# kwea123/nerf_pl

Hardware: NVIDIA H100
Metric: ray-samples/sec (coarse+fine) (higher is better)
Workload: dtype f16 (fp32 accumulate, fp32 encoding/compositing)

## Files before the change

include/nerf_pl_b200.h:

```cpp
#ifndef NERF_PL_B200_H_
#define NERF_PL_B200_H_

#include <stddef.h>
#include <stdint.h>

#ifdef __cplusplus
extern "C" {
#endif

#define NERFB200_ABI_VERSION 3

#define NERFB200_EINVAL (-1)
#define NERFB200_EUNSUPPORTED (-2)
#define NERFB200_EDEVICE (-3)

int nerfb200_abi_version(void);
const char* nerfb200_last_error(void);

size_t nerfb200_packed_bytes(void);
int nerfb200_pack_weights(const float* const params[24], void* packed, void* stream);
int nerfb200_pack_weights_pair(const float* const params_a[24], void* packed_a, const float* const params_b[24],
                               void* packed_b, void* stream);

typedef struct nerfb200_render_args {
// ... 68 lines not shown
int nerfb200_nerf_forward_train(const float* x, int64_t n, int64_t x_stride, const void* packed, void* ws, float* out,
                                void* stream);
int nerfb200_nerf_backward(const float* g_out, int64_t n, const void* packed, const float* const params[24], void* ws,
                           float* const grads[24], void* stream);

int nerfb200_query_sigma(const float* xyz, int64_t n, int64_t xyz_stride, const void* packed, float* sigma,
                         void* stream);

int nerfb200_mse_psnr(const float* rgb_coarse, const float* rgb_fine, const float* target, int64_t n_rays,
                      float* out4, void* stream);

int nerfb200_embed(const float* x, int64_t n, int32_t n_freqs, float* out, void* stream);

int nerfb200_searchsorted(const float* a, const float* v, int64_t* out, int64_t nrow_a,
                          int64_t nrow_v, int32_t ncol_a, int32_t ncol_v, int32_t side_right,
                          void* stream);

int nerfb200_sample_pdf(const float* bins, const float* weights, const float* u, int64_t n_rays,
                        int32_t n_weights, int32_t n_u, float* out, void* stream);

int nerfb200_composite(const float* sigmas, const float* rgbs, const float* z_vals,
                       const float* dirs, const float* noise, float noise_std, int32_t white_back,
                       int64_t n_rays, int32_t n_samples, float* weights, float* rgb, float* depth,
                       float* opacity, void* stream);

int nerfb200_generate_rays(int32_t H, int32_t W, float focal, const float c2w_host[12], float near, float far,
                           int32_t ndc, float* rays, void* stream);

int nerfb200_to_uint8(const float* src, int64_t n, uint8_t* dst, void* stream);

int64_t nerfb200_launch_count(void);
int nerfb200_check_status(void);
int nerfb200_sm_count(void);

#ifdef __cplusplus
}
#endif
#endif
```

nerf_pl_b200/_lib.py:

```python
from __future__ import annotations

import ctypes
import os
import subprocess
import threading
from ctypes import POINTER, c_char_p, c_float, c_int32, c_int64, c_size_t, c_void_p

_HERE = os.path.dirname(os.path.abspath(__file__))
CSRC = os.path.join(_HERE, "csrc")
LIB_PATH = os.path.join(_HERE, "libnerf_pl_b200.so")
if os.environ.get("NERFB200_LIB"):
    LIB_PATH = os.path.abspath(os.environ["NERFB200_LIB"])
SOURCES = ["capi.cu"]
HEADERS = ["ptx.cuh", "layout.h", "mlp_engine.cuh", "render_kernel.cuh", "aux_kernels.cuh", "bwd_kernels.cuh"]
NVCC_FLAGS = [
    "-gencode", "arch=compute_90a,code=sm_90a",
    "-O3", "-lineinfo", "-std=c++17",
    "--shared", "-Xcompiler", "-fPIC",
    "-diag-suppress", "550",
]

EXPORTS = [
    "nerfb200_abi_version",
    "nerfb200_last_error",
    "nerfb200_packed_bytes",
    "nerfb200_pack_weights",
    "nerfb200_pack_weights_pair",
    "nerfb200_render_rays",
    "nerfb200_render_rays_host",
    "nerfb200_nerf_forward",
    "nerfb200_nerf_train_workspace_bytes",
    "nerfb200_nerf_train_workspace_init",
    "nerfb200_nerf_forward_train",
    "nerfb200_nerf_backward",
    "nerfb200_embed",
    "nerfb200_searchsorted",
    "nerfb200_sample_pdf",
    "nerfb200_composite",
    "nerfb200_query_sigma",
    "nerfb200_mse_psnr",
    "nerfb200_train_workspace_bytes",
    "nerfb200_train_workspace_init",
    "nerfb200_render_backward",
    "nerfb200_adam_step",
    "nerfb200_generate_rays",
    "nerfb200_to_uint8",
    "nerfb200_launch_count",
    "nerfb200_check_status",
    "nerfb200_sm_count",
]

class RenderArgs(ctypes.Structure):

    _fields_ = [
        ("rays", c_void_p),
        ("n_rays", c_int64),
        ("ray_stride", c_int64),
        ("packed_coarse", c_void_p),
        ("packed_fine", c_void_p),
        ("n_samples", c_int32),
        ("n_importance", c_int32),
        ("use_disp", c_int32),
        ("perturb", c_float),
        ("noise_std", c_float),
        ("white_back", c_int32),
        ("test_time", c_int32),
        ("perturb_rand", c_void_p),
        ("noise_coarse", c_void_p),
        ("u_rand", c_void_p),
        ("noise_fine", c_void_p),
        ("rgb_coarse", c_void_p),
        ("depth_coarse", c_void_p),
        ("opacity_coarse", c_void_p),
        ("rgb_fine", c_void_p),
        ("depth_fine", c_void_p),
        ("opacity_fine", c_void_p),
        ("z_fine", c_void_p),
        ("weights_coarse", c_void_p),
        ("weights_fine", c_void_p),
        ("status", c_void_p),
        ("max_ctas", c_int32),
        ("z_coarse", c_void_p),
# ... 76 lines not shown
    lib.nerfb200_composite.argtypes = [c_void_p, c_void_p, c_void_p, c_void_p, c_void_p, c_float,
                                       c_int32, c_int64, c_int32, c_void_p, c_void_p, c_void_p,
                                       c_void_p, c_void_p]
    lib.nerfb200_query_sigma.argtypes = [c_void_p, c_int64, c_int64, c_void_p, c_void_p, c_void_p]
    lib.nerfb200_query_sigma.restype = c_int32
    lib.nerfb200_nerf_train_workspace_bytes.argtypes = [c_int64]
    lib.nerfb200_nerf_train_workspace_bytes.restype = c_size_t
    lib.nerfb200_nerf_train_workspace_init.argtypes = [c_void_p, c_size_t, c_int64, c_void_p]
    lib.nerfb200_nerf_train_workspace_init.restype = c_int32
    lib.nerfb200_nerf_forward_train.argtypes = [c_void_p, c_int64, c_int64, c_void_p, c_void_p, c_void_p, c_void_p]
    lib.nerfb200_nerf_forward_train.restype = c_int32
    lib.nerfb200_nerf_backward.argtypes = [c_void_p, c_int64, c_void_p, POINTER(c_void_p), c_void_p, POINTER(c_void_p),
                                           c_void_p]
    lib.nerfb200_nerf_backward.restype = c_int32
    lib.nerfb200_train_workspace_bytes.argtypes = [c_int64, c_int32, c_int32]
    lib.nerfb200_train_workspace_bytes.restype = c_size_t
    lib.nerfb200_train_workspace_init.argtypes = [c_void_p, c_size_t, c_int64, c_int32, c_int32, c_void_p]
    lib.nerfb200_train_workspace_init.restype = c_int32
    lib.nerfb200_render_backward.argtypes = [POINTER(BackwardArgs), c_void_p]
    lib.nerfb200_render_backward.restype = c_int32
    lib.nerfb200_adam_step.argtypes = [c_int32, POINTER(c_void_p), POINTER(c_void_p), POINTER(c_void_p), POINTER(c_void_p),
                                       POINTER(c_int64), c_float, c_float, c_float, c_float, c_float, c_int64, c_void_p]
    lib.nerfb200_adam_step.restype = c_int32
    lib.nerfb200_mse_psnr.argtypes = [c_void_p, c_void_p, c_void_p, c_int64, c_void_p, c_void_p]
    lib.nerfb200_mse_psnr.restype = c_int32
    lib.nerfb200_generate_rays.argtypes = [c_int32, c_int32, c_float, POINTER(c_float), c_float, c_float, c_int32,
                                           c_void_p, c_void_p]
    lib.nerfb200_generate_rays.restype = c_int32
    lib.nerfb200_to_uint8.argtypes = [c_void_p, c_int64, c_void_p, c_void_p]
    lib.nerfb200_to_uint8.restype = c_int32
    lib.nerfb200_check_status.restype = c_int32
    lib.nerfb200_launch_count.restype = c_int64
    lib.nerfb200_sm_count.restype = c_int32
    for name in ("nerfb200_pack_weights", "nerfb200_pack_weights_pair", "nerfb200_render_rays", "nerfb200_render_rays_host",
                 "nerfb200_nerf_forward", "nerfb200_embed", "nerfb200_searchsorted",
                 "nerfb200_sample_pdf", "nerfb200_composite"):
        getattr(lib, name).restype = c_int32


def load() -> ctypes.CDLL:
    global _lib
    with _lock:
        if _lib is None:
            if not os.path.exists(LIB_PATH):
                raise RuntimeError(
                    f"{LIB_PATH} is missing: run `python -c 'import __graft_entry__ as g; g.build()'` "
                    "(nerf_pl_b200 has no CPU fallback)")
            lib = ctypes.CDLL(LIB_PATH)
            _declare(lib)
            if lib.nerfb200_abi_version() != 3:
                raise RuntimeError("libnerf_pl_b200.so ABI version mismatch")
            _lib = lib
    return _lib


class NerfB200Error(RuntimeError):
    pass


def check(rc: int, what: str) -> None:
    if rc == 0:
        return
    msg = load().nerfb200_last_error().decode("utf-8", "replace")
    if rc in (-1, -2):
        raise ValueError(f"{what}: {msg}")
    raise NerfB200Error(f"{what}: {msg} (code {rc})")
# ... 1 lines not shown
```

nerf_pl_b200/csrc/capi.cu:

```cuda
#include <atomic>
#include <cstdio>
#include <cstdlib>
#include <cmath>
#include <cstring>
#include <mutex>
#include <vector>

#include "../../include/nerf_pl_b200.h"
#include "aux_kernels.cuh"
#include "bwd_kernels.cuh"

using namespace nerfb200;

namespace {

thread_local char g_err[512] = "";
std::atomic<long long> g_launches{0};

int fail(int code, const char* fmt, const char* detail = "") {
  std::snprintf(g_err, sizeof(g_err), fmt, detail);
  return code;
}
int cuda_fail(cudaError_t e, const char* where) {
  std::snprintf(g_err, sizeof(g_err), "%s: %s (%s)", where, cudaGetErrorString(e), cudaGetErrorName(e));
  return static_cast<int>(e);
}
#define CUDA_TRY(expr, where)                          \
  do {                                                 \
    cudaError_t e_ = (expr);                           \
    if (e_ != cudaSuccess) return cuda_fail(e_, where); \
  } while (0)

struct DeviceInfo {
  int sm_count = 0;
  int cc_major = 0, cc_minor = 0;
  bool attrs_set = false;
  int* status = nullptr;
  volatile int* status_host = nullptr;
  long long* timeline = nullptr;
};

struct EnvSwitches {
  unsigned flags = 0;
  int max_ctas = 0;
  int wg_plan = 1;
  int wg_copy = 32768;
  unsigned wg_exp = 0;
  int no_zero_copy = 0;
  EnvSwitches() {
    if (const char* v = std::getenv("NERFB200_NO_ZERO_COPY")) no_zero_copy = std::atoi(v);
    if (const char* v = std::getenv("NERFB200_WG_EXP")) wg_exp = static_cast<unsigned>(std::atoi(v));
    if (const char* v = std::getenv("NERFB200_WG_PLAN")) wg_plan = std::atoi(v);
    if (const char* v = std::getenv("NERFB200_WG_COPY")) wg_copy = std::atoi(v);
    if (const char* f = std::getenv("NERFB200_FLAGS")) flags = static_cast<unsigned>(std::strtoul(f, nullptr, 0));
    if (const char* mc = std::getenv("NERFB200_MAX_CTAS")) max_ctas = std::atoi(mc);
  }
};
const EnvSwitches& env_switches() {
  static const EnvSwitches e;
  return e;
}
std::mutex g_mu;
DeviceInfo g_dev[64];

int device_info(DeviceInfo** out) {
  int dev = 0;
  CUDA_TRY(cudaGetDevice(&dev), "cudaGetDevice");
  if (dev < 0 || dev >= 64) return fail(NERFB200_EDEVICE, "device ordinal out of range%s");
  std::lock_guard<std::mutex> lk(g_mu);
  DeviceInfo& d = g_dev[dev];
  if (d.sm_count == 0) {
    CUDA_TRY(cudaDeviceGetAttribute(&d.sm_count, cudaDevAttrMultiProcessorCount, dev), "attr sm");
    CUDA_TRY(cudaDeviceGetAttribute(&d.cc_major, cudaDevAttrComputeCapabilityMajor, dev), "attr cc");
    CUDA_TRY(cudaDeviceGetAttribute(&d.cc_minor, cudaDevAttrComputeCapabilityMinor, dev), "attr cc minor");
  }
  if (d.cc_major != 9 || d.cc_minor != 0) return fail(NERFB200_EDEVICE, "nerf_pl_b200 needs an sm_90 (H100) device%s");
  if (!d.attrs_set) {
    CUDA_TRY(cudaFuncSetAttribute(render_rays_kernel<false>, cudaFuncAttributeMaxDynamicSharedMemorySize,
                                  static_cast<int>(kSmemTotal)), "smem attr render");
    CUDA_TRY(cudaFuncSetAttribute(render_rays_kernel<true>, cudaFuncAttributeMaxDynamicSharedMemorySize,
                                  static_cast<int>(kSmemTotal)), "smem attr render(save)");
    CUDA_TRY(cudaFuncSetAttribute(mlp_forward_kernel<false>, cudaFuncAttributeMaxDynamicSharedMemorySize,
                                  static_cast<int>(kSmemTotal)), "smem attr mlp");
    CUDA_TRY(cudaFuncSetAttribute(mlp_forward_kernel<true>, cudaFuncAttributeMaxDynamicSharedMemorySize,
                                  static_cast<int>(kSmemTotal)), "smem attr mlp(save)");
    CUDA_TRY(cudaFuncSetAttribute(chain_bwd_kernel<false>, cudaFuncAttributeMaxDynamicSharedMemorySize,
                                  static_cast<int>(kChSmemTotal)), "smem attr chain");
    CUDA_TRY(cudaFuncSetAttribute(chain_bwd_kernel<true>, cudaFuncAttributeMaxDynamicSharedMemorySize,
                                  static_cast<int>(kChSmemTotal)), "smem attr chain (probe)");
    CUDA_TRY(cudaFuncSetAttribute(wgrad_kernel, cudaFuncAttributeMaxDynamicSharedMemorySize,
                                  static_cast<int>(kWgSmemTotal)), "smem attr wgrad");
    CUDA_TRY(cudaFuncSetAttribute(sample_pdf_kernel, cudaFuncAttributeMaxDynamicSharedMemorySize,
                                  static_cast<int>(kPdfWarps * (kPdfMaxWeights + 1) * sizeof(float))), "smem attr sample_pdf");
    int* hs = nullptr;
    CUDA_TRY(cudaHostAlloc(&hs, sizeof(int), cudaHostAllocMapped), "status alloc");
    *hs = 0;
    CUDA_TRY(cudaHostGetDevicePointer(&d.status, hs, 0), "status device pointer");
    d.status_host = hs;
    d.attrs_set = true;
  }
  *out = &d;
  return 0;
}

int check_sticky_status(DeviceInfo* d) {
  if (d->status_host == nullptr) return 0;
  const int st = *d->status_host;
  if (st == 0) return 0;
  *d->status_host = 0;
  if (st == 102)
    std::snprintf(g_err, sizeof(g_err), "an earlier training backward reported device status 102: a per-sample "
                  "gradient exceeded the fp16 range of its layer's scale, its weight gradients are wrong");
  else
    std::snprintf(g_err, sizeof(g_err), "an earlier nerf_pl_b200 kernel reported device status %d", st);
  return NERFB200_EDEVICE;
}

int check_render_shapes(const nerfb200_render_args* a) {
  if (a == nullptr) return fail(NERFB200_EINVAL, "args is NULL%s");
  if (a->n_rays < 0) return fail(NERFB200_EINVAL, "n_rays < 0%s");
  if (a->n_samples != 32 && a->n_samples != 64 && a->n_samples != 128)
    return fail(NERFB200_EUNSUPPORTED, "N_samples must be 32, 64 or 128%s");
  if (a->n_importance < 0 || (a->n_importance % 32) != 0)
    return fail(NERFB200_EUNSUPPORTED, "N_importance must be a multiple of 32%s");
  if (a->n_samples + a->n_importance > kMaxSf)
    return fail(NERFB200_EUNSUPPORTED, "N_samples + N_importance must be <= 192%s");
// ... 347 lines not shown
  add(slot(kJ1), kWgSlotFloats, ns(kJ1), g[0], linv + 8, 256, 63, 256, 63, 0, 1);
  add(slot(kJ1) + 65536, kWgSlotFloats, ns(kJ1), g[1], linv + 8, 1, 256, 256, 256, 0);
  const int hidden[6] = {kJ2, kJ3, kJ4, kJ6, kJ7, kJ8};
  const int layer[6] = {2, 3, 4, 6, 7, 8};
  for (int i = 0; i < 6; ++i) {
    const float* inv = linv + (9 - layer[i]);
    add(slot(hidden[i]), kWgSlotFloats, ns(hidden[i]), g[2 * (layer[i] - 1)], inv, 256, 256, 256, 256, 0, 1);
    add(slot(hidden[i]) + 65536, kWgSlotFloats, ns(hidden[i]), g[2 * (layer[i] - 1) + 1], inv, 1, 256, 256, 256, 0);
  }
  add(slot(kJ5a), kWgSlotFloats, ns(kJ5a), g[8], linv + 4, 256, 63, 256, 319, 0, 1);
  add(slot(kJ5b), kWgSlotFloats, ns(kJ5b), g[8], linv + 4, 256, 256, 256, 319, 63, 1);
  add(slot(kJ5a) + 65536, kWgSlotFloats, ns(kJ5a), g[9], linv + 4, 1, 256, 256, 256, 0);
  add(slot(kJ9), kWgSlotFloats, ns(kJ9), L.gWp[ps], linv, 128, 256, 128, 256, 0, 1);
  add(slot(kJ9) + 65536, kWgSlotFloats, ns(kJ9), L.gbp[ps], linv, 1, 128, 128, 128, 0);
  add(L.head_part[ps] + kHeadPartSigW, kHeadPartFloats, L.head_grid, g[20], nullptr, 1, 256, 256, 256, 0);
  add(L.head_part[ps] + kHeadPartSigB, kHeadPartFloats, L.head_grid, g[21], nullptr, 1, 1, 1, 1, 0);
  add(L.head_part[ps] + kHeadPartRgbW, kHeadPartFloats, L.head_grid, g[22], nullptr, 1, 384, 384, 384, 0);
  add(L.head_part[ps] + kHeadPartRgbB, kHeadPartFloats, L.head_grid, g[23], nullptr, 1, 3, 3, 3, 0);
  if (L.n_kinds == kNumJobKindsMlp)
    add(slot(kJDir), kWgSlotFloats, ns(kJDir), g[18], linv, 128, 27, 128, 283, 256, 1);
  else
    add(L.dir_part[ps], 128 * 27, kDirSlices, g[18], nullptr, 128, 27, 27, 283, 256);
}

}

extern "C" {

int nerfb200_abi_version(void) { return NERFB200_ABI_VERSION; }
const char* nerfb200_last_error(void) { return g_err; }
size_t nerfb200_packed_bytes(void) { return kPackedBytes; }
int64_t nerfb200_launch_count(void) { return g_launches.load(); }

int nerfb200_sm_count(void) {
  int dev = 0, n = 0;
  if (cudaGetDevice(&dev) != cudaSuccess) return 0;
  if (cudaDeviceGetAttribute(&n, cudaDevAttrMultiProcessorCount, dev) != cudaSuccess) return 0;
  return n;
}

static int fill_pack_params(PackParams* pp, const float* const params[24], void* packed) {
  if (!params || !packed) return fail(NERFB200_EINVAL, "pack_weights: NULL argument%s");
  if (reinterpret_cast<uintptr_t>(packed) & 15) return fail(NERFB200_EINVAL, "packed must be 16-byte aligned%s");
  for (int i = 0; i < kNumParams; ++i) {
    if (!params[i]) return fail(NERFB200_EINVAL, "pack_weights: NULL parameter tensor%s");
    pp->p[i] = params[i];
  }
  pp->out = static_cast<uint8_t*>(packed);
  pp->bwd_bf16 = kBwdBf16 ? 1 : 0;
  return 0;
}

static int launch_pack(const PackParams2& pp2, int n_nets, void* stream) {
  const long long total = kHalfRegionBytes / 2 + kF32Count + static_cast<long long>(kNumSlicesBwd) * 256 * 64;
  const int threads = 256;
  const int blocks = static_cast<int>((total + threads - 1) / threads);
  pack_weights_kernel<<<dim3(blocks, n_nets), threads, 0, static_cast<cudaStream_t>(stream)>>>(pp2);
  g_launches++;
  CUDA_TRY(cudaGetLastError(), "pack_weights launch");
  return 0;
}

int nerfb200_pack_weights(const float* const params[24], void* packed, void* stream) {
  PackParams2 pp2;
  int rc = fill_pack_params(&pp2.net[0], params, packed);
  if (rc) return rc;
// ... 62 lines not shown
    make_train_layout(&L, static_cast<uint8_t*>(a->train_workspace), a->n_rays, a->n_samples, a->n_importance, d->sm_count);
    p.train = 1;
    p.tr[0] = L.pass[0];
    p.tr[1] = L.pass[1];
    if (!p.z_coarse) p.z_coarse = L.pass[0].z;
    else return fail(NERFB200_EINVAL, "z_coarse is owned by the workspace in training mode%s");
    if (a->n_importance > 0) {
      if (p.z_fine) return fail(NERFB200_EINVAL, "z_fine is owned by the workspace in training mode%s");
      p.z_fine = L.pass[1].z;
    }
    if (a->target) {
      p.target = a->target;
      p.loss_out = a->loss_out;
      p.loss_part = L.loss_part;
      p.loss_counter = L.loss_counter;
    }
  }
  p.flags = env_switches().flags;
  p.timeline = nullptr;
#ifdef NERFB200_TIMELINE
  if (p.flags & 2u) {
    if (!d->timeline) {
      CUDA_TRY(cudaMalloc(&d->timeline, 3 * kTlMax * 2 * sizeof(long long)), "timeline alloc");
    }
    CUDA_TRY(cudaMemsetAsync(d->timeline, 0, 3 * kTlMax * 2 * sizeof(long long), static_cast<cudaStream_t>(stream)), "timeline memset");
    p.timeline = d->timeline;
  }
#endif
  const int n_groups = (p.n_rays + 1) / 2;
  int ctas = d->sm_count;
  if (a->max_ctas > 0 && a->max_ctas < ctas) ctas = a->max_ctas;
  if (env_switches().max_ctas > 0 && env_switches().max_ctas < ctas) ctas = env_switches().max_ctas;
  if (n_groups < ctas) ctas = n_groups;
  if (save)
    render_rays_kernel<true><<<ctas, kRenderThreads, kSmemTotal, static_cast<cudaStream_t>(stream)>>>(p);
  else
    render_rays_kernel<false><<<ctas, kRenderThreads, kSmemTotal, static_cast<cudaStream_t>(stream)>>>(p);
  g_launches++;
  CUDA_TRY(cudaGetLastError(), "render_rays launch");
  return 0;
}

int nerfb200_render_rays_host(const nerfb200_render_args* h, void* stream_v) {
  int rc = check_render_shapes(h);
  if (rc) return rc;
  if (h->n_rays == 0) return 0;
  cudaStream_t stream = static_cast<cudaStream_t>(stream_v);
  if (h->train_workspace || h->target || h->z_coarse)
    return fail(NERFB200_EINVAL, "render_rays_host: train_workspace / target / z_coarse are device-only%s");
  {
    bool all_mapped = true;
    auto mapped = [&](const void* p, const void** dp) -> bool {
      *dp = nullptr;
      if (!p) return true;
      cudaPointerAttributes attr;
      if (cudaPointerGetAttributes(&attr, p) != cudaSuccess) { (void)cudaGetLastError(); return false; }
      if ((attr.type == cudaMemoryTypeHost || attr.type == cudaMemoryTypeDevice || attr.type == cudaMemoryTypeManaged) &&
          attr.devicePointer != nullptr) {
        *dp = attr.devicePointer;
        return true;
      }
      return false;
    };
    nerfb200_render_args a = *h;
    const void* dp = nullptr;
#define NERFB200_MAP(field, type)                                          \
    all_mapped = all_mapped && mapped(h->field, &dp);                      \
    a.field = static_cast<type>(const_cast<void*>(dp));
    NERFB200_MAP(rays, const float*)
    NERFB200_MAP(perturb_rand, const float*)
    NERFB200_MAP(noise_coarse, const float*)
// ... 597 lines not shown
```

nerf_pl_b200/csrc/mlp_engine.cuh:

```cuda
#pragma once
#include <cuda_fp16.h>

#include "layout.h"
#include "ptx.cuh"

namespace nerfb200 {

constexpr int kConsumerWGs = 2;
constexpr int kConsumerThreads = kConsumerWGs * 128;
constexpr int kConsumerWarp0 = 4;
constexpr int kProducerWarp = 0;
constexpr int kThreads = (1 + kConsumerWGs) * 128;
constexpr int kRegsAux = 56;
constexpr int kRegsConsumer = 224;
static_assert(kRegsAux + 2 * kRegsConsumer <= 3 * 168, "setmaxnreg budget");
constexpr int kWgBar0 = 4;
#ifndef NERFB200_STAGES
#define NERFB200_STAGES 3
#endif
constexpr int kStages = NERFB200_STAGES;

constexpr uint32_t kSmemEnc = 0;
constexpr uint32_t kSmemRing = 16384;
constexpr uint32_t kSmemEnc1 = kSmemRing + kStages * kSliceBytes256;
constexpr uint32_t kSmemConsts = kSmemEnc1 + 16384;
constexpr uint32_t kConstFloats = kF32WDirPart;
constexpr uint32_t kConstRegion = 24576;
constexpr uint32_t kSmemScratch = kSmemConsts + kConstRegion;
static_assert(2 * kConstFloats * 4 <= kConstRegion, "constants of two networks must fit");
static_assert(kSmemEnc1 % 1024 == 0 && kSmemConsts % 1024 == 0, "SWIZZLE_128B tiles need 1024-byte alignment");
constexpr uint32_t kSmemTotal = 232448;
constexpr uint32_t kScratchBytes = kSmemTotal - kSmemScratch;

struct Barriers {
  uint64_t full[kStages];
  uint64_t empty[kStages];
};
static_assert(sizeof(Barriers) % 16 == 0, "Barriers must keep 16-byte alignment of what follows");

struct RingState {
  uint32_t stage = 0, phase = 0;
  __device__ __forceinline__ void advance() {
    if (++stage == kStages) { stage = 0; phase ^= 1; }
  }
};

__device__ __forceinline__ bool engine_setup(uint8_t* smem, Barriers* bars) {
  if ((smem_u32(smem) & 1023u) != 0) return false;
  if (threadIdx.x == 0) {
    for (int i = 0; i < kStages; ++i) {
      mbar_init(smem_u32(&bars->full[i]), 1);
      mbar_init(smem_u32(&bars->empty[i]), kConsumerWGs * 4);
    }
    fence_mbar_init();
  }
  __syncthreads();
  return true;
}

__device__ __forceinline__ void load_consts(uint8_t* smem, int slot, const uint8_t* __restrict__ blob) {
  if (blob == nullptr) return;
  const float4* src = reinterpret_cast<const float4*>(blob + kHalfRegionBytes);
  float4* dst = reinterpret_cast<float4*>(smem + kSmemConsts) + slot * (kConstFloats / 4);
  for (uint32_t i = threadIdx.x; i < kConstFloats / 4; i += blockDim.x) dst[i] = __ldg(src + i);
}
__device__ __forceinline__ const float* consts_ptr(uint8_t* smem, int slot) {
  return reinterpret_cast<const float*>(smem + kSmemConsts) + slot * kConstFloats;
}

__device__ __forceinline__ void produce_tile(RingState& rs, uint8_t* smem, Barriers* bars,
                                             const uint8_t* __restrict__ blob, bool sigma_only,
                                             bool dir_slice) {
  const int n256 = sigma_only ? kNumSlicesSigmaOnly : kNumSlices256;
  for (int i = 0; i < n256; ++i) {
    mbar_wait(smem_u32(&bars->empty[rs.stage]), rs.phase ^ 1, 1);
    const uint32_t full = smem_u32(&bars->full[rs.stage]);
    const uint32_t dst = smem_u32(smem + kSmemRing + rs.stage * kSliceBytes256);
    mbar_arrive_expect_tx(full, kSliceBytes256);
    const uint8_t* src = blob + static_cast<size_t>(i) * kSliceBytes256;
#pragma unroll
    for (int c = 0; c < 4; ++c) bulk_g2s(dst + c * 8192, src + c * 8192, 8192, full);
    rs.advance();
  }
  if (!sigma_only) {
    const int n128 = dir_slice ? 5 : 4;
    for (int i = 0; i < n128; ++i) {
      mbar_wait(smem_u32(&bars->empty[rs.stage]), rs.phase ^ 1, 2);
      const uint32_t full = smem_u32(&bars->full[rs.stage]);
      const uint32_t dst = smem_u32(smem + kSmemRing + rs.stage * kSliceBytes256);
      mbar_arrive_expect_tx(full, kSliceBytes128);
      const uint8_t* src = blob + kOffDir + static_cast<size_t>(i) * kSliceBytes128;
#pragma unroll
      for (int c = 0; c < 2; ++c) bulk_g2s(dst + c * 8192, src + c * 8192, 8192, full);
      rs.advance();
    }
  }
}

struct WgCtx {
  uint8_t* smem;
  Barriers* bars;
  RingState rs;
  int wg, wi, lane, q;
  int row[2];
  const float* cst;
  uint8_t* save_act;
  uint2* save_mask;
  uint8_t* save_d;
  long long save_n;
  long long grow[2];
};

__device__ __forceinline__ void wg_bar(const WgCtx& c) { named_bar_sync(kWgBar0 + c.wg, 128); }

__device__ __forceinline__ void release_stage(const WgCtx& c, uint32_t stage) {
  __syncwarp();
  if (c.lane == 0) mbar_arrive(smem_u32(&c.bars->empty[stage]));
}

template <int kMode>
__device__ __forceinline__ void mma_layer(WgCtx& c, float (&acc)[128], const uint32_t (&h)[64], uint64_t a_desc,
                                          uint64_t ring_desc) {
  constexpr int n_slices = (kMode == 0) ? 1 : (kMode == 5) ? 2 : (kMode == 2 || kMode == 4) ? 5 : 4;
  constexpr bool kN128 = (kMode == 3 || kMode == 4);
  const uint32_t full0 = smem_u32(&c.bars->full[0]);
  wgmma_fence();
  uint32_t prev = 0;
#pragma unroll
  for (int s = 0; s < n_slices; ++s) {
    const bool from_smem = (kMode == 0) || (kMode == 5) || (kMode == 2 && s == 0) || (kMode == 4 && s == 4);
    const int kb = (kMode == 2) ? s - 1 : s;
    const uint32_t stage = c.rs.stage;
    mbar_wait(full0 + 8u * stage, c.rs.phase, 4);
    const uint64_t bdesc = ring_desc + static_cast<uint64_t>(stage * (kSliceBytes256 >> 4));
    const uint64_t adesc = a_desc + ((kMode == 5) ? static_cast<uint64_t>(kb * (16384 >> 4)) : 0ull);
#pragma unroll
    for (int j = 0; j < 4; ++j) {
      const uint32_t sd = (s | j) != 0 ? 1u : 0u;
      if (from_smem) {
        if (kN128) wgmma_n128_ss(reinterpret_cast<float(&)[64]>(acc), adesc + 2 * j, bdesc + 2 * j, sd);
        else wgmma_n256_ss(acc, adesc + 2 * j, bdesc + 2 * j, sd);
      } else {
        const uint32_t(&a)[4] = *reinterpret_cast<const uint32_t(*)[4]>(&h[4 * (4 * kb + j)]);
        if (kN128) wgmma_n128_rs(reinterpret_cast<float(&)[64]>(acc), a, bdesc + 2 * j, sd);
        else wgmma_n256_rs(acc, a, bdesc + 2 * j, sd);
      }
    }
    wgmma_commit();
    if (s > 0) {
      wgmma_wait<1>();
// ... 142 lines not shown
  if (!kSigmaOnly) {
    if (kDirSlice) {
      write_dir_rows(c, enc_off, *ds);
      mma_layer<4>(c, acc, h, enc_desc, ring_desc);
    } else {
      mma_layer<3>(c, acc, h, enc_desc, ring_desc);
    }
    epi_dir<kSave>(c, acc, dbias, c.cst + kF32WRgb, rgb);
  }
#pragma unroll
  for (int s = 0; s < 2; ++s) {
    sig[s] = quad_sum(sig[s]);
    if (!kSigmaOnly) {
      rgb[s][0] = quad_sum(rgb[s][0]);
      rgb[s][1] = quad_sum(rgb[s][1]);
      rgb[s][2] = quad_sum(rgb[s][2]);
    }
  }
}

__device__ __forceinline__ void wg_init(WgCtx& c, uint8_t* smem, Barriers* bars) {
  const int ct = threadIdx.x - kConsumerWarp0 * 32;
  c.smem = smem;
  c.bars = bars;
  c.wg = ct >> 7;
  c.wi = (ct >> 5) & 3;
  c.lane = ct & 31;
  c.q = c.lane & 3;
  c.row[0] = 64 * c.wg + 16 * c.wi + (c.lane >> 2);
  c.row[1] = c.row[0] + 8;
  c.cst = nullptr;
  c.save_act = nullptr; c.save_mask = nullptr; c.save_d = nullptr; c.save_n = 0;
  c.grow[0] = c.grow[1] = -1;
}

__device__ __forceinline__ float sigmoid_ref(float x) { return 1.f / (1.f + expf(-x)); }

}
```

nerf_pl_b200/csrc/ptx.cuh:

```cuda
#pragma once
#include <cstdint>
#include <cuda_runtime.h>

namespace nerfb200 {

__device__ int g_watchdog_code = 0;

__device__ __forceinline__ void report_fault(int* status, int code) {
  if (status == nullptr) return;
  *reinterpret_cast<volatile int*>(status) = code;
  __threadfence_system();
}

__device__ __forceinline__ uint32_t smem_u32(const void* p) {
  return static_cast<uint32_t>(__cvta_generic_to_shared(p));
}

__device__ __forceinline__ void mbar_init(uint32_t bar, uint32_t count) {
  asm volatile("mbarrier.init.shared::cta.b64 [%0], %1;" ::"r"(bar), "r"(count) : "memory");
}
__device__ __forceinline__ void fence_mbar_init() {
  asm volatile("fence.mbarrier_init.release.cluster;" ::: "memory");
}
__device__ __forceinline__ void mbar_arrive(uint32_t bar) {
// ... 14 lines not shown
      : "=r"(ok)
      : "r"(bar), "r"(parity)
      : "memory");
  return ok != 0;
}
__device__ __forceinline__ void mbar_wait(uint32_t bar, uint32_t parity, int code) {
  if (mbar_try_wait(bar, parity)) return;
#ifdef NERFB200_SANITIZE
  while (!mbar_try_wait(bar, parity)) {}
  return;
#endif
  const long long t0 = clock64();
  while (!mbar_try_wait(bar, parity)) {
    if (clock64() - t0 > 4000000000LL) {
      g_watchdog_code = code;
      __threadfence_system();
      __trap();
    }
  }
}

__device__ __forceinline__ void fence_proxy_async() {
  asm volatile("fence.proxy.async.shared::cta;" ::: "memory");
}

__device__ __forceinline__ void bulk_g2s(uint32_t dst_smem, const void* src, uint32_t bytes,
                                         uint32_t bar) {
  asm volatile(
      "cp.async.bulk.shared::cluster.global.mbarrier::complete_tx::bytes [%0], [%1], %2, [%3];"
      ::"r"(dst_smem), "l"(src), "r"(bytes), "r"(bar)
      : "memory");
}

__device__ __forceinline__ void bulk_s2g(void* gdst, uint32_t smem_src, uint32_t bytes) {
  asm volatile("cp.async.bulk.global.shared::cta.bulk_group [%0], [%1], %2;" ::"l"(gdst), "r"(smem_src), "r"(bytes)
               : "memory");
}
__device__ __forceinline__ void bulk_commit() { asm volatile("cp.async.bulk.commit_group;" ::: "memory"); }
__device__ __forceinline__ void bulk_wait_read() { asm volatile("cp.async.bulk.wait_group.read 0;" ::: "memory"); }
template <int N>
__device__ __forceinline__ void bulk_wait_read_n() {
  asm volatile("cp.async.bulk.wait_group.read %0;" ::"n"(N) : "memory");
}
__device__ __forceinline__ void bulk_wait_all() { asm volatile("cp.async.bulk.wait_group 0;" ::: "memory"); }
__device__ __forceinline__ void named_bar_sync(int id, int n_threads) {
  asm volatile("bar.sync %0, %1;" ::"r"(id), "r"(n_threads) : "memory");
}

template <int kRegs>
__device__ __forceinline__ void regs_dec() { asm volatile("setmaxnreg.dec.sync.aligned.u32 %0;" ::"n"(kRegs)); }
template <int kRegs>
__device__ __forceinline__ void regs_inc() { asm volatile("setmaxnreg.inc.sync.aligned.u32 %0;" ::"n"(kRegs)); }

__device__ __forceinline__ void wgmma_fence() { asm volatile("wgmma.fence.sync.aligned;" ::: "memory"); }
__device__ __forceinline__ void wgmma_commit() { asm volatile("wgmma.commit_group.sync.aligned;" ::: "memory"); }
template <int N>
__device__ __forceinline__ void wgmma_wait() { asm volatile("wgmma.wait_group.sync.aligned %0;" ::"n"(N) : "memory"); }
template <int N>
__device__ __forceinline__ void reg_fence(float (&d)[N]) {
#pragma unroll
  for (int i = 0; i < N; ++i) asm volatile("" : "+f"(d[i])::"memory");
}

__device__ __forceinline__ void wgmma_n256_rs(float (&d)[128], const uint32_t (&a)[4], uint64_t bdesc, uint32_t scale_d) {
  asm volatile(
      "{\n\t.reg .pred p;\n\t"
// ... 82 lines not shown
```

nerf_pl_b200/csrc/render_kernel.cuh:

```cuda
#pragma once
#include "mlp_engine.cuh"

namespace nerfb200 {

constexpr int kMaxSc = 128;
constexpr int kMaxSf = 192;
constexpr int kMaxImp = kMaxSf - 32;
constexpr int kMaxRows = 2 * kMaxSf;

struct PassBufs {
  long long n;
  long long n_pad;
  int S;
  uint8_t* enc;
  uint8_t* act;
  uint2* mask;
  uint8_t* d;
  float* sigma;
  float* rgb;
  float* z;
  float* dsigma;
  float* dprergb;
  uint8_t* dd;
  uint8_t* dpre;
// ... 290 lines not shown
  bool fine;
  int g = 0, phase = 0, t = 0, q = 0;
  __device__ __forceinline__ TileSeq(int G_, int my_n_, int Sc_, int Sf_, bool fine_)
      : G(G_), my_n(my_n_), Sc(Sc_), Sf(Sf_), fine(fine_) {}
  __device__ __forceinline__ int nr(int gg) const { return min(2, my_n - 2 * gg); }
  __device__ __forceinline__ static int tiles_of(int n_r, int S) { return (n_r * S + 127) >> 7; }
  __device__ __forceinline__ bool next(Tile& o) {
    while (g <= G) {
      if (phase == 0) {
        const int nt = (g < G) ? tiles_of(nr(g), Sc) : 0;
        if (t < nt) { o = Tile{q, g, 0, t, t + 1 == nt}; ++t; ++q; return true; }
        phase = 1; t = 0;
      } else {
        const int nt = (fine && g >= 1) ? tiles_of(nr(g - 1), Sf) : 0;
        if (t < nt) { o = Tile{q, g - 1, 1, t, t + 1 == nt}; ++t; ++q; return true; }
        phase = 0; t = 0; ++g;
      }
    }
    return false;
  }
};

template <bool kSave>
__global__ void __launch_bounds__(kRenderThreads, 1) render_rays_kernel(const RenderParams p) {
  extern __shared__ __align__(1024) uint8_t smem[];
  RenderScratch* sc = reinterpret_cast<RenderScratch*>(smem + kSmemScratch);
  Barriers* bars = &sc->bars;
  if (threadIdx.x == 0) {
    for (int b = 0; b < 2; ++b) {
      mbar_init(smem_u32(&sc->enc_full[b]), kHandoffPerThread ? kHelperThreads : kHelperWarps);
      mbar_init(smem_u32(&sc->out_full[b]), kHandoffPerThread ? kConsumerThreads : kConsumerThreads / 32);
    }
  }
  if (!engine_setup(smem, bars)) {
    if (threadIdx.x == 0) report_fault(p.status, 101);
    return;
  }
  load_consts(smem, 0, p.net_coarse);
  load_consts(smem, 1, p.net_fine);
  __syncthreads();
  const int warp = threadIdx.x >> 5;
  const int lane = threadIdx.x & 31;
  const int Sc = p.n_samples;
  const int K = p.n_importance;
  const int Sf = Sc + K;
  const bool fine = K > 0;
  const bool coarse_sigma_only = p.test_time != 0;
  const int per_cta = p.n_rays / static_cast<int>(gridDim.x), rem_cta = p.n_rays % static_cast<int>(gridDim.x);
  const int my_lo = static_cast<int>(blockIdx.x) * per_cta + min(static_cast<int>(blockIdx.x), rem_cta);
  const int my_n = per_cta + (static_cast<int>(blockIdx.x) < rem_cta ? 1 : 0);
  const int n_groups = (my_n + 1) >> 1;
  TileSeq seq(n_groups, my_n, Sc, Sf, fine);
  Tile tl;

  if (warp >= kConsumerWarp0) {
    regs_inc<kRegsConsumer>();
    WgCtx c;
    wg_init(c, smem, bars);
    while (seq.next(tl)) {
      const int b = tl.q & 1;
      const int pass = tl.pass;
      const int S = pass ? Sf : Sc;
      const bool valid1 = seq.nr(tl.g) == 2;
      const int ray0 = my_lo + 2 * tl.g;
      const bool sigma_only = (pass == 0) && coarse_sigma_only;
      const uint32_t enc_off = b ? kSmemEnc1 : kSmemEnc;
      c.cst = consts_ptr(smem, pass);
      c.save_act = kSave ? p.tr[pass].act : nullptr;
      c.save_mask = kSave ? p.tr[pass].mask : nullptr;
      c.save_d = kSave ? p.tr[pass].d : nullptr;
      c.save_n = kSave ? p.tr[pass].n_pad : 0;
      const GroupState& gs = sc->gs[tl.g % kGroupSlots];
      const float* dbias[2];
#pragma unroll
      for (int s = 0; s < 2; ++s) {
        const int gr = tl.tile * 128 + c.row[s];
        const int r = (gr >= S) ? 1 : 0;
        c.grow[s] = (gr < 2 * S && (r == 0 || valid1)) ? static_cast<long long>(ray0 + r) * S + (gr - r * S) : -1;
        dbias[s] = gs.dirbias[pass][r];
      }
      mbar_wait(smem_u32(&sc->enc_full[b]), static_cast<uint32_t>(tl.q >> 1) & 1u, 7);
      if (kSave && c.wi < 2 && c.lane == 0) {
        const int grp = 64 * c.wg + 32 * c.wi;
        const int gr0 = tl.tile * 128 + grp;
        const int r0 = (gr0 >= S) ? 1 : 0;
        if (gr0 < 2 * S && (r0 == 0 || valid1)) {
          const long long g0 = static_cast<long long>(ray0 + r0) * S + (gr0 - r0 * S);
          bulk_s2g(p.tr[pass].enc + tiled_block_off(static_cast<unsigned long long>(g0 >> 6), 0, 1) + (g0 & 63) * 128,
                   smem_u32(smem + enc_off + grp * 128), 4096);
          bulk_commit();
        }
      }
      float sig[2], rgb[2][3];
      if (sigma_only) wg_tile<true, false, kSave>(c, enc_off, dbias, nullptr, sig, rgb);
      else wg_tile<false, false, kSave>(c, enc_off, dbias, nullptr, sig, rgb);
#pragma unroll
      for (int s = 0; s < 2; ++s) {
        const int row = c.row[s];
        const long long grow = c.grow[s];
        if (c.q == 0) {
          const float sg = c.cst[kF32BSigma] + sig[s];
          sc->out_sigma[b][row] = sg;
          if (kSave && grow >= 0) p.tr[pass].sigma[grow] = sg;
        } else if (!sigma_only) {
          const int ch = c.q - 1;
          const float part = (ch == 0) ? rgb[s][0] : (ch == 1) ? rgb[s][1] : rgb[s][2];
          const float col = sigmoid_ref(c.cst[kF32BRgb + ch] + part);
          sc->out_rgb[b][ch][row] = col;
          if (kSave && grow >= 0) p.tr[pass].rgb[grow * 3 + ch] = col;
        }
      }
      if (kSave && c.wi < 2 && c.lane == 0) bulk_wait_read();
      if (kHandoffPerThread) {
        mbar_arrive(smem_u32(&sc->out_full[b]));
      } else {
        __syncwarp();
        if (c.lane == 0) mbar_arrive(smem_u32(&sc->out_full[b]));
      }
    }
    if (kSave) bulk_wait_all();
  } else if (warp == kProducerWarp) {
    regs_dec<kRegsAux>();
    if (lane == 0) {
      RingState rs;
      while (seq.next(tl))
        produce_tile(rs, smem, bars, tl.pass ? p.net_fine : p.net_coarse, tl.pass == 0 && coarse_sigma_only, false);
    }
  } else if (warp < kHelperWarp0 + kHelperWarps) {
    regs_dec<kRegsAux>();
    const int ht = threadIdx.x - kHelperWarp0 * 32;
    const int hw = ht >> 5;
    TileSeq cons_seq(n_groups, my_n, Sc, Sf, fine);
    Tile tc;
    float loss_c = 0.f, loss_f = 0.f;
    int consumed = 0;
    int cpos0 = 0, cpos1 = 0, cpos2 = 0;

    auto consume = [&](const Tile& tt) {
      const int b = tt.q & 1;
      const int pass = tt.pass;
      const int S = pass ? Sf : Sc;
      const bool valid1 = seq.nr(tt.g) == 2;
      const int ray0 = my_lo + 2 * tt.g;
      const int rid[2] = {ray0, valid1 ? ray0 + 1 : ray0};
      const bool sigma_only = (pass == 0) && coarse_sigma_only;
      GroupState& gs = sc->gs[tt.g % kGroupSlots];
      mbar_wait(smem_u32(&sc->out_full[b]), static_cast<uint32_t>(tt.q >> 1) & 1u, 8);
      for (int row = ht; row < 128; row += kHelperThreads) {
        const int gr = tt.tile * 128 + row;
        if (gr < 2 * S) {
          gs.sigma[gr] = sc->out_sigma[b][row];
          if (!sigma_only) {
            gs.rgb[0][gr] = sc->out_rgb[b][0][row];
            gs.rgb[1][gr] = sc->out_rgb[b][1][row];
            gs.rgb[2][gr] = sc->out_rgb[b][2][row];
          }
        }
      }
      helper_bar();
// ... 214 lines not shown
      }
    }
    while (cons_seq.next(tc)) consume(tc);
    if (p.target != nullptr) {
      float* lsum = sc->lsum;
      helper_bar();
      if (lane == 0 && hw < 2) { lsum[2 * hw] = loss_c; lsum[2 * hw + 1] = loss_f; }
      helper_bar();
      if (ht == 0) {
        p.loss_part[2 * blockIdx.x] = lsum[0] + lsum[2];
        p.loss_part[2 * blockIdx.x + 1] = lsum[1] + lsum[3];
        __threadfence();
        const unsigned ticket = atomicAdd(p.loss_counter, 1u);
        if (ticket == gridDim.x - 1) {
          __threadfence();
          double sc_ = 0.0, sf_ = 0.0;
          for (unsigned i = 0; i < gridDim.x; ++i) {
            sc_ += static_cast<double>(*reinterpret_cast<volatile float*>(p.loss_part + 2 * i));
            sf_ += static_cast<double>(*reinterpret_cast<volatile float*>(p.loss_part + 2 * i + 1));
          }
          const double ne = 3.0 * static_cast<double>(p.n_rays);
          const float mc = static_cast<float>(sc_ / ne), mf = static_cast<float>(sf_ / ne);
          p.loss_out[0] = mc;
          p.loss_out[1] = fine ? mf : 0.f;
          p.loss_out[2] = fine ? mc + mf : mc;
          p.loss_out[3] = -10.f * log10f(fine ? mf : mc);
          *p.loss_counter = 0u;
        }
      }
    }
  } else {
    regs_dec<kRegsAux>();
  }
}

}
```

Measured before the change: 543.4 million.

## Launch render kernel in CTA pairs and multicast weight slices across cluster

Renders are launched as 2-CTA clusters when the CTA count and ray split are even. Each CTA's producer fetches half of every weight slice and multicasts it to both CTAs, and consumers release ring stages on both their own and the peer's empty barrier. This halves the L2-to-SMEM weight traffic per CTA, at the cost of cross-CTA coupling where the slower CTA stalls its partner. The ring also grows from three to four stages, and the constant region is shrunk to its exact size to make room.

```diff
diff --git a/include/nerf_pl_b200.h b/include/nerf_pl_b200.h
--- a/include/nerf_pl_b200.h
+++ b/include/nerf_pl_b200.h
@@ -124,6 +124,7 @@
 int64_t nerfb200_launch_count(void);
 int nerfb200_check_status(void);
 int nerfb200_sm_count(void);
+int nerfb200_last_render_cluster(void);
 
 #ifdef __cplusplus
 }
diff --git a/nerf_pl_b200/_lib.py b/nerf_pl_b200/_lib.py
--- a/nerf_pl_b200/_lib.py
+++ b/nerf_pl_b200/_lib.py
@@ -48,6 +48,7 @@
     "nerfb200_launch_count",
     "nerfb200_check_status",
     "nerfb200_sm_count",
+    "nerfb200_last_render_cluster",
 ]
 
 class RenderArgs(ctypes.Structure):
@@ -190,6 +191,7 @@
     lib.nerfb200_check_status.restype = c_int32
     lib.nerfb200_launch_count.restype = c_int64
     lib.nerfb200_sm_count.restype = c_int32
+    lib.nerfb200_last_render_cluster.restype = c_int32
     for name in ("nerfb200_pack_weights", "nerfb200_pack_weights_pair", "nerfb200_render_rays", "nerfb200_render_rays_host",
                  "nerfb200_nerf_forward", "nerfb200_embed", "nerfb200_searchsorted",
                  "nerfb200_sample_pdf", "nerfb200_composite"):
diff --git a/nerf_pl_b200/csrc/capi.cu b/nerf_pl_b200/csrc/capi.cu
--- a/nerf_pl_b200/csrc/capi.cu
+++ b/nerf_pl_b200/csrc/capi.cu
@@ -15,6 +15,7 @@
 namespace {
 
 thread_local char g_err[512] = "";
+thread_local int g_render_cluster = 0;
 std::atomic<long long> g_launches{0};
 
 int fail(int code, const char* fmt, const char* detail = "") {
@@ -34,6 +35,7 @@
 struct DeviceInfo {
   int sm_count = 0;
   int cc_major = 0, cc_minor = 0;
+  int max_pairs = 0;
   bool attrs_set = false;
   int* status = nullptr;
   volatile int* status_host = nullptr;
@@ -43,6 +45,7 @@
 struct EnvSwitches {
   unsigned flags = 0;
   int max_ctas = 0;
+  int cluster = 0;
   int wg_plan = 1;
   int wg_copy = 32768;
   unsigned wg_exp = 0;
@@ -54,6 +57,7 @@
     if (const char* v = std::getenv("NERFB200_WG_COPY")) wg_copy = std::atoi(v);
     if (const char* f = std::getenv("NERFB200_FLAGS")) flags = static_cast<unsigned>(std::strtoul(f, nullptr, 0));
     if (const char* mc = std::getenv("NERFB200_MAX_CTAS")) max_ctas = std::atoi(mc);
+    if (const char* v = std::getenv("NERFB200_CLUSTER")) cluster = std::atoi(v);
   }
 };
 const EnvSwitches& env_switches() {
@@ -92,6 +96,23 @@
                                   static_cast<int>(kWgSmemTotal)), "smem attr wgrad");
     CUDA_TRY(cudaFuncSetAttribute(sample_pdf_kernel, cudaFuncAttributeMaxDynamicSharedMemorySize,
                                   static_cast<int>(kPdfWarps * (kPdfMaxWeights + 1) * sizeof(float))), "smem attr sample_pdf");
+    {
+      cudaLaunchConfig_t qc = {};
+      cudaLaunchAttribute qa[1];
+      qa[0].id = cudaLaunchAttributeClusterDimension;
+      qa[0].val.clusterDim.x = 2;
+      qa[0].val.clusterDim.y = 1;
+      qa[0].val.clusterDim.z = 1;
+      qc.gridDim = dim3(2 * (d.sm_count / 2));
+      qc.blockDim = dim3(kRenderThreads);
+      qc.dynamicSmemBytes = kSmemTotal;
+      qc.attrs = qa;
+      qc.numAttrs = 1;
+      int n0 = 0, n1 = 0;
+      CUDA_TRY(cudaOccupancyMaxActiveClusters(&n0, render_rays_kernel<false>, &qc), "cluster occupancy render");
+      CUDA_TRY(cudaOccupancyMaxActiveClusters(&n1, render_rays_kernel<true>, &qc), "cluster occupancy render(save)");
+      d.max_pairs = n0 < n1 ? n0 : n1;
+    }
     int* hs = nullptr;
     CUDA_TRY(cudaHostAlloc(&hs, sizeof(int), cudaHostAllocMapped), "status alloc");
     *hs = 0;
@@ -505,6 +526,8 @@
 size_t nerfb200_packed_bytes(void) { return kPackedBytes; }
 int64_t nerfb200_launch_count(void) { return g_launches.load(); }
 
+int nerfb200_last_render_cluster(void) { return g_render_cluster; }
+
 int nerfb200_sm_count(void) {
   int dev = 0, n = 0;
   if (cudaGetDevice(&dev) != cudaSuccess) return 0;
@@ -633,11 +656,32 @@
   if (a->max_ctas > 0 && a->max_ctas < ctas) ctas = a->max_ctas;
   if (env_switches().max_ctas > 0 && env_switches().max_ctas < ctas) ctas = env_switches().max_ctas;
   if (n_groups < ctas) ctas = n_groups;
-  if (save)
-    render_rays_kernel<true><<<ctas, kRenderThreads, kSmemTotal, static_cast<cudaStream_t>(stream)>>>(p);
-  else
-    render_rays_kernel<false><<<ctas, kRenderThreads, kSmemTotal, static_cast<cudaStream_t>(stream)>>>(p);
-  g_launches++;
+  const bool pair = ctas % 2 == 0 && (p.n_rays % ctas) % 2 == 0 && d->max_pairs >= ctas / 2 &&
+                    env_switches().cluster != 1;
+  if (pair) {
+    cudaLaunchConfig_t cfg = {};
+    cudaLaunchAttribute attr[1];
+    attr[0].id = cudaLaunchAttributeClusterDimension;
+    attr[0].val.clusterDim.x = 2;
+    attr[0].val.clusterDim.y = 1;
+    attr[0].val.clusterDim.z = 1;
+    cfg.gridDim = dim3(ctas);
+    cfg.blockDim = dim3(kRenderThreads);
+    cfg.dynamicSmemBytes = kSmemTotal;
+    cfg.stream = static_cast<cudaStream_t>(stream);
+    cfg.attrs = attr;
+    cfg.numAttrs = 1;
+    g_launches++;
+    if (save) CUDA_TRY(cudaLaunchKernelEx(&cfg, render_rays_kernel<true>, p), "render_rays launch (cluster 2)");
+    else CUDA_TRY(cudaLaunchKernelEx(&cfg, render_rays_kernel<false>, p), "render_rays launch (cluster 2)");
+  } else {
+    if (save)
+      render_rays_kernel<true><<<ctas, kRenderThreads, kSmemTotal, static_cast<cudaStream_t>(stream)>>>(p);
+    else
+      render_rays_kernel<false><<<ctas, kRenderThreads, kSmemTotal, static_cast<cudaStream_t>(stream)>>>(p);
+    g_launches++;
+  }
+  g_render_cluster = pair ? 2 : 1;
   CUDA_TRY(cudaGetLastError(), "render_rays launch");
   return 0;
 }
diff --git a/nerf_pl_b200/csrc/mlp_engine.cuh b/nerf_pl_b200/csrc/mlp_engine.cuh
--- a/nerf_pl_b200/csrc/mlp_engine.cuh
+++ b/nerf_pl_b200/csrc/mlp_engine.cuh
@@ -16,7 +16,7 @@
 static_assert(kRegsAux + 2 * kRegsConsumer <= 3 * 168, "setmaxnreg budget");
 constexpr int kWgBar0 = 4;
 #ifndef NERFB200_STAGES
-#define NERFB200_STAGES 3
+#define NERFB200_STAGES 4
 #endif
 constexpr int kStages = NERFB200_STAGES;
 
@@ -25,7 +25,7 @@
 constexpr uint32_t kSmemEnc1 = kSmemRing + kStages * kSliceBytes256;
 constexpr uint32_t kSmemConsts = kSmemEnc1 + 16384;
 constexpr uint32_t kConstFloats = kF32WDirPart;
-constexpr uint32_t kConstRegion = 24576;
+constexpr uint32_t kConstRegion = 2 * kConstFloats * 4;
 constexpr uint32_t kSmemScratch = kSmemConsts + kConstRegion;
 static_assert(2 * kConstFloats * 4 <= kConstRegion, "constants of two networks must fit");
 static_assert(kSmemEnc1 % 1024 == 0 && kSmemConsts % 1024 == 0, "SWIZZLE_128B tiles need 1024-byte alignment");
@@ -45,12 +45,12 @@
   }
 };
 
-__device__ __forceinline__ bool engine_setup(uint8_t* smem, Barriers* bars) {
+__device__ __forceinline__ bool engine_setup(uint8_t* smem, Barriers* bars, uint32_t n_cta = 1) {
   if ((smem_u32(smem) & 1023u) != 0) return false;
   if (threadIdx.x == 0) {
     for (int i = 0; i < kStages; ++i) {
       mbar_init(smem_u32(&bars->full[i]), 1);
-      mbar_init(smem_u32(&bars->empty[i]), kConsumerWGs * 4);
+      mbar_init(smem_u32(&bars->empty[i]), n_cta * kConsumerWGs * 4);
     }
     fence_mbar_init();
   }
@@ -70,28 +70,40 @@
 
 __device__ __forceinline__ void produce_tile(RingState& rs, uint8_t* smem, Barriers* bars,
                                              const uint8_t* __restrict__ blob, bool sigma_only,
-                                             bool dir_slice) {
+                                             bool dir_slice, uint32_t rank = 0, uint32_t n_cta = 1) {
   const int n256 = sigma_only ? kNumSlicesSigmaOnly : kNumSlices256;
   for (int i = 0; i < n256; ++i) {
-    mbar_wait(smem_u32(&bars->empty[rs.stage]), rs.phase ^ 1, 1);
+    mbar_wait(smem_u32(&bars->empty[rs.stage]), rs.phase ^ 1, n_cta > 1 ? 11 : 1);
     const uint32_t full = smem_u32(&bars->full[rs.stage]);
     const uint32_t dst = smem_u32(smem + kSmemRing + rs.stage * kSliceBytes256);
     mbar_arrive_expect_tx(full, kSliceBytes256);
     const uint8_t* src = blob + static_cast<size_t>(i) * kSliceBytes256;
-#pragma unroll
-    for (int c = 0; c < 4; ++c) bulk_g2s(dst + c * 8192, src + c * 8192, 8192, full);
+    if (n_cta > 1) {
+#pragma unroll
+      for (int c = 0; c < 2; ++c) {
+        const uint32_t cc = 2 * rank + c;
+        bulk_g2s_multicast(dst + cc * 8192, src + cc * 8192, 8192, full, 0x3);
+      }
+    } else {
+#pragma unroll
+      for (int c = 0; c < 4; ++c) bulk_g2s(dst + c * 8192, src + c * 8192, 8192, full);
+    }
     rs.advance();
   }
   if (!sigma_only) {
     const int n128 = dir_slice ? 5 : 4;
     for (int i = 0; i < n128; ++i) {
-      mbar_wait(smem_u32(&bars->empty[rs.stage]), rs.phase ^ 1, 2);
+      mbar_wait(smem_u32(&bars->empty[rs.stage]), rs.phase ^ 1, n_cta > 1 ? 12 : 2);
       const uint32_t full = smem_u32(&bars->full[rs.stage]);
       const uint32_t dst = smem_u32(smem + kSmemRing + rs.stage * kSliceBytes256);
       mbar_arrive_expect_tx(full, kSliceBytes128);
       const uint8_t* src = blob + kOffDir + static_cast<size_t>(i) * kSliceBytes128;
-#pragma unroll
-      for (int c = 0; c < 2; ++c) bulk_g2s(dst + c * 8192, src + c * 8192, 8192, full);
+      if (n_cta > 1) {
+        bulk_g2s_multicast(dst + rank * 8192, src + rank * 8192, 8192, full, 0x3);
+      } else {
+#pragma unroll
+        for (int c = 0; c < 2; ++c) bulk_g2s(dst + c * 8192, src + c * 8192, 8192, full);
+      }
       rs.advance();
     }
   }
@@ -109,13 +121,18 @@
   uint8_t* save_d;
   long long save_n;
   long long grow[2];
+  uint32_t n_cta;
+  uint32_t peer_empty0;
 };
 
 __device__ __forceinline__ void wg_bar(const WgCtx& c) { named_bar_sync(kWgBar0 + c.wg, 128); }
 
 __device__ __forceinline__ void release_stage(const WgCtx& c, uint32_t stage) {
   __syncwarp();
-  if (c.lane == 0) mbar_arrive(smem_u32(&c.bars->empty[stage]));
+  if (c.lane == 0) {
+    mbar_arrive(smem_u32(&c.bars->empty[stage]));
+    if (c.n_cta > 1) mbar_arrive_cluster(c.peer_empty0 + 8u * stage);
+  }
 }
 
 template <int kMode>
@@ -324,6 +341,8 @@
   c.cst = nullptr;
   c.save_act = nullptr; c.save_mask = nullptr; c.save_d = nullptr; c.save_n = 0;
   c.grow[0] = c.grow[1] = -1;
+  c.n_cta = 1;
+  c.peer_empty0 = 0;
 }
 
 __device__ __forceinline__ float sigmoid_ref(float x) { return 1.f / (1.f + expf(-x)); }
diff --git a/nerf_pl_b200/csrc/ptx.cuh b/nerf_pl_b200/csrc/ptx.cuh
--- a/nerf_pl_b200/csrc/ptx.cuh
+++ b/nerf_pl_b200/csrc/ptx.cuh
@@ -70,6 +70,36 @@
       : "memory");
 }
 
+__device__ __forceinline__ void bulk_g2s_multicast(uint32_t dst_smem, const void* src, uint32_t bytes, uint32_t bar,
+                                                   uint16_t cta_mask) {
+  asm volatile(
+      "cp.async.bulk.shared::cluster.global.mbarrier::complete_tx::bytes.multicast::cluster [%0], [%1], %2, [%3], %4;"
+      ::"r"(dst_smem), "l"(src), "r"(bytes), "r"(bar), "h"(cta_mask)
+      : "memory");
+}
+
+__device__ __forceinline__ uint32_t cluster_ctarank() {
+  uint32_t r;
+  asm volatile("mov.u32 %0, %%cluster_ctarank;" : "=r"(r));
+  return r;
+}
+__device__ __forceinline__ uint32_t cluster_nctarank() {
+  uint32_t n;
+  asm volatile("mov.u32 %0, %%cluster_nctarank;" : "=r"(n));
+  return n;
+}
+__device__ __forceinline__ uint32_t mapa_shared(uint32_t smem_addr, uint32_t rank) {
+  uint32_t r;
+  asm volatile("mapa.shared::cluster.u32 %0, %1, %2;" : "=r"(r) : "r"(smem_addr), "r"(rank));
+  return r;
+}
+__device__ __forceinline__ void mbar_arrive_cluster(uint32_t cluster_bar) {
+  asm volatile("mbarrier.arrive.shared::cluster.b64 _, [%0];" ::"r"(cluster_bar) : "memory");
+}
+__device__ __forceinline__ void cluster_sync() {
+  asm volatile("barrier.cluster.arrive.release;\n\tbarrier.cluster.wait.acquire;" ::: "memory");
+}
+
 __device__ __forceinline__ void bulk_s2g(void* gdst, uint32_t smem_src, uint32_t bytes) {
   asm volatile("cp.async.bulk.global.shared::cta.bulk_group [%0], [%1], %2;" ::"l"(gdst), "r"(smem_src), "r"(bytes)
                : "memory");
diff --git a/nerf_pl_b200/csrc/render_kernel.cuh b/nerf_pl_b200/csrc/render_kernel.cuh
--- a/nerf_pl_b200/csrc/render_kernel.cuh
+++ b/nerf_pl_b200/csrc/render_kernel.cuh
@@ -346,10 +346,12 @@
       mbar_init(smem_u32(&sc->out_full[b]), kHandoffPerThread ? kConsumerThreads : kConsumerThreads / 32);
     }
   }
-  if (!engine_setup(smem, bars)) {
+  const uint32_t n_cta = cluster_nctarank();
+  if (!engine_setup(smem, bars, n_cta)) {
     if (threadIdx.x == 0) report_fault(p.status, 101);
     return;
   }
+  if (n_cta > 1) cluster_sync();
   load_consts(smem, 0, p.net_coarse);
   load_consts(smem, 1, p.net_fine);
   __syncthreads();
@@ -371,6 +373,8 @@
     regs_inc<kRegsConsumer>();
     WgCtx c;
     wg_init(c, smem, bars);
+    c.n_cta = n_cta;
+    if (n_cta > 1) c.peer_empty0 = mapa_shared(smem_u32(&bars->empty[0]), cluster_ctarank() ^ 1u);
     while (seq.next(tl)) {
       const int b = tl.q & 1;
       const int pass = tl.pass;
@@ -437,8 +441,10 @@
     regs_dec<kRegsAux>();
     if (lane == 0) {
       RingState rs;
+      const uint32_t rank = cluster_ctarank();
       while (seq.next(tl))
-        produce_tile(rs, smem, bars, tl.pass ? p.net_fine : p.net_coarse, tl.pass == 0 && coarse_sigma_only, false);
+        produce_tile(rs, smem, bars, tl.pass ? p.net_fine : p.net_coarse, tl.pass == 0 && coarse_sigma_only, false,
+                     rank, n_cta);
     }
   } else if (warp < kHelperWarp0 + kHelperWarps) {
     regs_dec<kRegsAux>();
@@ -719,6 +725,7 @@
   } else {
     regs_dec<kRegsAux>();
   }
-}
-
-}
+  if (n_cta > 1) cluster_sync();
+}
+
+}
```

Result: no change. 544.9 million (median of 6 runs) (+0.3%).
